# YushenLi807/WWW24-RAT

Measured on AMD Instinct MI355X. Metric: training samples/sec at B=4096, K=10 retrieved, d=64; 1/2/4/8 MI355X, higher is better.
Workload: dtype f32; 1 GPU; synthetic_F20_V1M_K10_d64_B4096; fields=20, vocab_rows=1000000, retrieved=10, embedding_dim=64, batch_per_gpu=4096, global_batch=4096, heads=8, dim_head=10, depth=4, scale_dim=2, step=fwd+bwd+clip+adam, embedding_grad=atomic, sync_batch_norm=False, parallelism=dp1

## Files before the change

www24-rat_amd/csrc/attn.hip:

```cpp
#include "rat_device.h"
#include "../../include/rat_hip.h"

#include <cstdlib>
#include <initializer_list>

namespace {

constexpr int ATT_THREADS = 512;
constexpr int ATT_WAVES = ATT_THREADS / 64;
constexpr int ATT_ROWS = 64;
constexpr int ATT_MT = ATT_ROWS / 16;
constexpr int DH_MAX = 16;
constexpr int QSLOTS = 8;
constexpr int OSLOTS = 4;
constexpr int FAST_INNER = 80;
constexpr int fast_heads(int tdh) { return tdh > 0 ? FAST_INNER / tdh : 0; }
constexpr int CORE_UNROLL = 3;

struct AttnArgs {
    const float* x;
    const float* dy;
    float* y;
    const float* res;
    const float* add;
    int add_lds;
    float out_scale;
    float* o_save;
    float* lse_save;
    const float* ln_g;
    const float* ln_b;
    const float* w_qkv;
    const float* w_out;
    const float* b_out;
    float* slabs;
    int64_t slab_stride;
    int64_t nseq, q_div, hi_stride, lo_stride, pos_stride;
    int64_t nchunks;
    int L, nsq_chunk;
    int nq;
    int d, heads, dh;
    float eps, scale;
    int vec_x, vec_wqkv, vec_wout;
    RatDrop drop;
    int groups;
    int64_t group_tok;
    unsigned long long* prof;
};

struct AttnGeom {
    int D, I, Q3, D16, I16, Q16, ldx, ldq, ldt;
    __host__ __device__ AttnGeom(int d, int heads, int dh) {
        D = d;
        I = heads * dh;
        Q3 = 3 * I;
        D16 = (D + 15) / 16 * 16;
        I16 = (I + 15) / 16 * 16;
        Q16 = (Q3 + 15) / 16 * 16;
        ldx = D16 + 4;
        ldq = Q16 + 4;
        ldt = (D16 > I16 ? D16 : I16) + 4;
    }
    size_t fwd_smem() const { return (size_t)ATT_ROWS * (ldx + ldq) * 4 + 2 * ATT_ROWS * 8; }
    size_t bwd_smem(int heads) const {
        return (size_t)ATT_ROWS * (2 * ldx + ldq + 2 * ldt) * 4 + (size_t)ATT_ROWS * (2 + 2 * heads) * 4 + 2 * ATT_ROWS * 8;
    }
    int64_t slab_floats() const { return (int64_t)Q3 * D + (int64_t)D * I + 3 * (int64_t)D; }
};

__device__ __forceinline__ int64_t seq_token(const AttnArgs& a, int64_t q, int p) {
    if (a.nseq <= 0x7fffffffLL && a.q_div <= 0x7fffffffLL) {
        const unsigned qq = (unsigned)q, dv = (unsigned)a.q_div, hi = qq / dv;
        return (int64_t)hi * a.hi_stride + (int64_t)(qq - hi * dv) * a.lo_stride + (int64_t)p * a.pos_stride;
    }
    return (q / a.q_div) * a.hi_stride + (q % a.q_div) * a.lo_stride + (int64_t)p * a.pos_stride;
}

__device__ __forceinline__ void map_rows(const AttnArgs& a, int64_t chunk, int64_t* rowtok, int& nsq, int& rows) {
    const int64_t q0 = chunk * a.nsq_chunk;
    const int64_t left = a.nseq - q0;
    nsq = left < a.nsq_chunk ? (int)left : a.nsq_chunk;
    rows = nsq * a.L;
    if (threadIdx.x < ATT_ROWS) {
        const int r = threadIdx.x;
        rowtok[r] = r < rows ? seq_token(a, q0 + r / a.L, r % a.L) : (int64_t)-1;
    }
// ... 935 lines not shown
    RAT_REQUIRE(d <= 128, "embedding_dim > 128 is not supported by this kernel");
    RAT_REQUIRE(map->L >= 1 && map->L <= ATT_ROWS, "sequence length (K+1 or F+1) must be in [1, 64]");
    RAT_REQUIRE(map->nseq >= 1 && map->q_div >= 1, "bad seq map");
    const AttnGeom g(d, heads, dim_head);
    RAT_REQUIRE(g.fwd_smem() <= 160 * 1024, "heads*dim_head too large for the LDS tile (forward)");
    if (backward) {
        RAT_REQUIRE(g.bwd_smem(heads) <= 160 * 1024, "heads*dim_head too large for the LDS tile (backward)");
        RAT_REQUIRE((g.Q16 / 16) * (g.D16 / 16) <= QSLOTS * ATT_WAVES,
                    "3*heads*dim_head x embedding_dim exceeds the in-register dW_qkv accumulator budget");
        RAT_REQUIRE((g.D16 / 16) * (g.I16 / 16) <= OSLOTS * ATT_WAVES,
                    "embedding_dim x heads*dim_head exceeds the in-register dW_out accumulator budget");
    }
    return 0;
}

bool aligned16(const void* p) { return (reinterpret_cast<uintptr_t>(p) & 15) == 0; }

void fill_common(AttnArgs& a, const RatAttnParams* w, const RatSeqMap* map, int d, int heads, int dim_head,
                 float ln_eps) {
    a.ln_g = w->ln_g;
    a.ln_b = w->ln_b;
    a.w_qkv = w->w_qkv;
    a.w_out = w->w_out;
    a.b_out = w->b_out;
    a.nseq = map->nseq;
    a.q_div = map->q_div;
    a.hi_stride = map->hi_stride;
    a.lo_stride = map->lo_stride;
    a.pos_stride = map->pos_stride;
    a.L = map->L;
    a.nq = (map->queries > 0 && map->queries < map->L) ? map->queries : map->L;
    a.nsq_chunk = ATT_ROWS / map->L;
    a.nchunks = (map->nseq + a.nsq_chunk - 1) / a.nsq_chunk;
    a.d = d;
    a.heads = heads;
    a.dh = dim_head;
    a.eps = ln_eps;
    a.scale = 1.0f / sqrtf((float)dim_head);
    a.out_scale = 1.0f;
    const int I = heads * dim_head;
    a.vec_wqkv = (d % 4 == 0) && aligned16(w->w_qkv);
    a.vec_wout = (I % 4 == 0) && aligned16(w->w_out);
    a.prof = rat_prof_buffer();
}

bool aligned8(const void* p) { return (reinterpret_cast<uintptr_t>(p) & 7) == 0; }

int fast_dim(const AttnArgs& a, std::initializer_list<const void*> ptrs) {
    if (!((a.dh == 10 || a.dh == 20) && a.heads == fast_heads(a.dh)) || a.w_out == nullptr) return 0;
    for (const void* p : ptrs)
        if (p != nullptr && !aligned16(p)) return 0;
    if (!aligned16(a.w_qkv) || !aligned16(a.w_out)) return 0;
    return (a.d == 64 || a.d == 16) ? a.d : 0;
}

}

extern "C" int rat_attn_fwd(const float* x, float* y, float* o_save, float* lse_save, const RatAttnParams* w_host,
                            const RatSeqMap* map_host, int d, int heads, int dim_head, float ln_eps, void* stream) {
    return rat_attn_fwd_ex(x, x, y, o_save, lse_save, w_host, map_host, d, heads, dim_head, 0.f, 1.f, ln_eps, 0.f, 0, RAT_ARITH_F32,
                           nullptr, 0, stream);
}

static bool b3_dim(int d) { return d == B3_D || d == 40 || d == 48 || d == 56; }
static bool b3_geom(int d, int heads, int dim_head) {
    return (b3_dim(d) && heads == B3_H && dim_head == B3_DH) || (d == B3_D && heads == 4 && dim_head == 2 * B3_DH);
}
static bool b3_shape(int d, int heads, int dim_head, const RatAttnParams* w) {
    return b3_geom(d, heads, dim_head) && w->w_out != nullptr;
}
static bool b3_ph_fits(int L, int nsq_chunk, int heads = B3_H) { return (size_t)nsq_chunk * heads * L * L * 4 <= (size_t)3 * B3_XP; }
static int b3_matrix_core(int L) {
    const int k = rat_knob(RAT_KNOB_ATTN_BWD_CORE_MFMA);
    if (L > 48 || k == 0) return 0;
    if (L > 32) return (k == 1 || L >= 40) ? 13 : 0;
    return (k == 1 || L >= 28) ? (L > 16 ? 2 : 1) : 0;
}
static int b3_fwd_matrix_core(int L, int nq) {
    const int k = rat_knob(RAT_KNOB_ATTN_FWD_CORE_MFMA);
    if (L > 48 || nq < L || k == 3) return 0;
    if (k != 2 && !((L >= 28 && L <= 32) || L >= 40)) return 0;
    return L > 32 ? 3 : (L > 16 ? 2 : 1);
}
static bool b3_ph_enabled() {
    return rat_knob(RAT_KNOB_ATTN_BWD_PH) != 0;
}
static int b3_nvalid(int d) { return d == B3_D ? 0 : d; }
static bool b3_off32_ok(const RatSeqMap* m) {
    if (m->hi_stride < 0 || m->lo_stride < 0 || m->pos_stride < 0) return false;
    const int64_t qd = m->q_div, hi = (m->nseq - 1) / qd, lo = m->nseq - 1 < qd - 1 ? m->nseq - 1 : qd - 1;
    const double max_tok = (double)hi * (double)m->hi_stride + (double)lo * (double)m->lo_stride + (double)(m->L - 1) * (double)m->pos_stride;
    return (max_tok + 1.0) * (double)(B3_I * 4) < 4294967296.0;
}

extern "C" size_t rat_attn_fwd_workspace(int d, int heads, int dim_head) {
    return b3_geom(d, heads, dim_head) ? B3_W_QKV + B3_W_OUT : 0;
}

extern "C" size_t rat_attn_planes_bytes(int d, int heads, int dim_head) {
    return b3_geom(d, heads, dim_head) ? B3_W_BYTES : 0;
}
extern "C" int rat_attn_split_jobs(const RatAttnParams* w_host, int d, int heads, int dim_head, void* planes, RatSplitJob* jobs_out) {
    RAT_REQUIRE(w_host && jobs_out, "null pointer");
    if (!b3_shape(d, heads, dim_head, w_host) || planes == nullptr) return 0;
    RAT_REQUIRE(aligned16(planes) && w_host->w_qkv, "planes must be 16-byte aligned");
    char* ws = static_cast<char*>(planes);
    jobs_out[0] = RatSplitJob{w_host->w_qkv, ws, B3_Q3, d, d, 0, 0, 0};
    jobs_out[1] = RatSplitJob{w_host->w_out, ws + B3_W_QKV, B3_I, d, B3_I, 1, 0, 0};
    jobs_out[2] = RatSplitJob{w_host->w_qkv, ws + B3_W_QKV + B3_W_OUTT, B3_D, B3_Q3, d, 1, 0, b3_nvalid(d)};
    jobs_out[3] = RatSplitJob{w_host->w_out, ws + B3_W_QKV + B3_W_OUTT + B3_W_QKVT, B3_D, B3_I, B3_I, 0, 0, b3_nvalid(d)};
    return 4;
}

extern "C" int rat_attn_fwd_ex(const float* x, const float* res, float* y, float* o_save, float* lse_save,
                               const RatAttnParams* w_host, const RatSeqMap* map_host, int d, int heads, int dim_head,
                               float softmax_scale, float out_scale, float ln_eps, float dropout_p, uint64_t dropout_seed,
                               int arith, float* workspace, size_t workspace_bytes, void* stream) {
    if (check_dims(map_host, d, heads, dim_head, false)) return -1;
    RAT_REQUIRE(x && y && w_host && w_host->ln_g && w_host->ln_b && w_host->w_qkv, "null pointer");
    RAT_REQUIRE(w_host->w_out != nullptr || heads * dim_head == d, "missing w_out");
    AttnArgs a{};
    fill_common(a, w_host, map_host, d, heads, dim_head, ln_eps);
    if (softmax_scale > 0.f) a.scale = softmax_scale;
    a.out_scale = out_scale;
    a.res = res;
    a.x = x;
    a.y = y;
    a.o_save = o_save;
    a.lse_save = lse_save;
    a.vec_x = (d % 4 == 0) && aligned16(x) && aligned16(y) && aligned16(res);
    const AttnGeom g(d, heads, dim_head);
    const bool ct_shape = dim_head == 10 && ((d == 10 && (heads == 8 || heads == 2)) || (d == 16 && heads == 2));
    const size_t smem = g.fwd_smem() + (ct_shape ? ct_weight_floats(g) * sizeof(float) : 0);
    const int per_cu = (int)((160 * 1024) / smem) >= 2 ? 2 : 1;
    const unsigned blocks = (unsigned)(a.nchunks < rat_max_blocks() * per_cu ? a.nchunks : rat_max_blocks() * per_cu);
    RAT_REQUIRE(dropout_p >= 0.f && dropout_p < 1.f, "dropout_p must be in [0, 1)");
    if (dropout_p > 0.f && w_host->w_out != nullptr)
        a.drop = RatDrop{dropout_seed, (uint32_t)((double)dropout_p * 4294967296.0), 1.0f / (1.0f - dropout_p), w_host->drop_seed_dev};
    const int fast = fast_dim(a, {x, y, res, o_save, lse_save});
    const bool plain = res == x && out_scale == 1.0f && a.drop.threshold == 0;
    const bool have_planes = w_host->planes != nullptr && aligned16(w_host->planes);
    const bool dpad = d != B3_D && b3_dim(d) && heads == fast_heads(dim_head) && aligned16(x) && aligned16(y) && aligned16(res) &&
                      aligned16(o_save) && aligned16(lse_save) && aligned16(w_host->w_qkv) && aligned16(w_host->w_out);
    if (arith == RAT_ARITH_BF16X3 && (fast == 64 || dpad) && b3_shape(d, heads, dim_head, w_host) && b3_off32_ok(map_host) &&
        (have_planes || (workspace != nullptr && workspace_bytes >= B3_W_QKV + B3_W_OUT && aligned16(workspace)))) {
        const char* p_qkv;
        const char* p_out;
        if (have_planes) {
            p_qkv = static_cast<const char*>(w_host->planes);
            p_out = p_qkv + B3_W_QKV + B3_W_OUTT + B3_W_QKVT;
        } else {
            char* ws = reinterpret_cast<char*>(workspace);
            if (rat_launch_split_weights(w_host->w_qkv, B3_Q3, d, d, 0, ws, stream) ||
                rat_launch_split_weights(w_host->w_out, B3_D, B3_I, B3_I, 0, ws + B3_W_QKV, stream, 0, b3_nvalid(d))) return -1;
            p_qkv = ws;
            p_out = ws + B3_W_QKV;
        }
        Attn3W W{};
        W.qkv = RatWPlanes{reinterpret_cast<const rat_u4*>(p_qkv), 2};
        W.out = RatWPlanes{reinterpret_cast<const rat_u4*>(p_out), 3};
        const unsigned b3_blocks = (unsigned)(a.nchunks < rat_max_blocks() ? a.nchunks : rat_max_blocks());
        if (heads == 4) {
            RAT_LAUNCH((attn_fwd3_kernel<true, false, false, false, 0, 4>), b3_blocks, ATT_THREADS, b3_fwd_smem(), stream, a, W);
            return rat_check_launch("rat_attn_fwd (bf16x3, 4 heads)");
        }
        if (dpad) {
            if (plain && a.nq < a.L) RAT_LAUNCH((attn_fwd3_kernel<false, true, true>), b3_blocks, ATT_THREADS, b3_fwd_smem(), stream, a, W);
            else if (plain) RAT_LAUNCH((attn_fwd3_kernel<false, false, true>), b3_blocks, ATT_THREADS, b3_fwd_smem(), stream, a, W);
            else RAT_LAUNCH((attn_fwd3_kernel<true, false, true>), b3_blocks, ATT_THREADS, b3_fwd_smem(), stream, a, W);
        } else if (plain && a.nq < a.L) RAT_LAUNCH((attn_fwd3_kernel<false, true>), b3_blocks, ATT_THREADS, b3_fwd_smem(), stream, a, W);
        else if (plain && b3_fwd_matrix_core(a.L, a.nq) == 3)
            RAT_LAUNCH((attn_fwd3_kernel<false, false, false, false, 3>), b3_blocks, ATT_THREADS, b3_fwd_smem(), stream, a, W);
        else if (plain && b3_fwd_matrix_core(a.L, a.nq) == 2)
            RAT_LAUNCH((attn_fwd3_kernel<false, false, false, false, 2>), b3_blocks, ATT_THREADS, b3_fwd_smem(), stream, a, W);
        else if (plain && b3_fwd_matrix_core(a.L, a.nq) == 1)
            RAT_LAUNCH((attn_fwd3_kernel<false, false, false, false, 1>), b3_blocks, ATT_THREADS, b3_fwd_smem(), stream, a, W);
        else if (plain) RAT_LAUNCH((attn_fwd3_kernel<false>), b3_blocks, ATT_THREADS, b3_fwd_smem(), stream, a, W);
        else if (b3_fwd_matrix_core(a.L, a.L) == 3)
            RAT_LAUNCH((attn_fwd3_kernel<true, false, false, false, 3>), b3_blocks, ATT_THREADS, b3_fwd_smem(), stream, a, W);
        else if (b3_fwd_matrix_core(a.L, a.L) == 2)
            RAT_LAUNCH((attn_fwd3_kernel<true, false, false, false, 2>), b3_blocks, ATT_THREADS, b3_fwd_smem(), stream, a, W);
        else RAT_LAUNCH((attn_fwd3_kernel<true>), b3_blocks, ATT_THREADS, b3_fwd_smem(), stream, a, W);
        return rat_check_launch("rat_attn_fwd (bf16x3)");
    }
    const bool head_vec = aligned8(o_save);
    RAT_REQUIRE(head_vec || dim_head <= DH_MAX, "o_save must be 8-byte aligned for dim_head 20");
    if (!head_vec) RAT_LAUNCH((attn_fwd_kernel<0, 0>), blocks, ATT_THREADS, smem, stream, a);
    else if (fast == 64 && dim_head == 10 && plain) RAT_LAUNCH((attn_fwd_kernel<64, 10, false>), blocks, ATT_THREADS, smem, stream, a);
    else if (fast == 64 && dim_head == 10) RAT_LAUNCH((attn_fwd_kernel<64, 10>), blocks, ATT_THREADS, smem, stream, a);
    else if (fast == 16 && dim_head == 10) RAT_LAUNCH((attn_fwd_kernel<16, 10>), blocks, ATT_THREADS, smem, stream, a);
    else if (fast == 64 && dim_head == 20) RAT_LAUNCH((attn_fwd_kernel<64, 20>), blocks, ATT_THREADS, smem, stream, a);
    else if (dim_head == 20) RAT_LAUNCH((attn_fwd_kernel<0, 20>), blocks, ATT_THREADS, smem, stream, a);
    else if (dim_head == 10 && d == 10 && heads == 8) RAT_LAUNCH((attn_fwd_kernel<0, 10, true, 2, 8, 10>), blocks, ATT_THREADS, smem, stream, a);
    else if (dim_head == 10 && d == 10 && heads == 2) RAT_LAUNCH((attn_fwd_kernel<0, 10, true, 2, 2, 10>), blocks, ATT_THREADS, smem, stream, a);
    else if (dim_head == 10 && d == 16 && heads == 2) RAT_LAUNCH((attn_fwd_kernel<0, 10, true, 2, 2, 16>), blocks, ATT_THREADS, smem, stream, a);
    else if (dim_head == 10 && d <= 16) RAT_LAUNCH((attn_fwd_kernel<0, 10, true, 2>), blocks, ATT_THREADS, smem, stream, a);
    else if (dim_head == 10) RAT_LAUNCH((attn_fwd_kernel<0, 10>), blocks, ATT_THREADS, smem, stream, a);
    else RAT_LAUNCH((attn_fwd_kernel<0, 0>), blocks, ATT_THREADS, smem, stream, a);
    return rat_check_launch("rat_attn_fwd");
}

static int b3_groups(int d, int heads, int dim_head) {
    return (d == B3_D && dim_head == B3_DH && heads > B3_H && heads % B3_H == 0 && heads / B3_H <= 8) ? heads / B3_H : 0;
}
static int wide_heads(int dim_head) { return dim_head == WG_DH ? WG_H : (dim_head == 2 * WG_DH ? WG_H / 2 : 0); }
static int wide_groups(int d, int heads, int dim_head) {
    const int wh = wide_heads(dim_head);
    return (d >= 1 && d <= 16 && wh > 0 && heads > wh && heads % wh == 0 && heads / wh <= 8) ? heads / wh : 0;
}
extern "C" int rat_attn_groups_supported(int d, int heads, int dim_head) {
    if (b3_groups(d, heads, dim_head)) return 1;
    const int G = wide_groups(d, heads, dim_head);
    return G == 0 ? 0 : (G <= WG_MAXG ? 3 : 1);
}
extern "C" size_t rat_attn_groups_planes_bytes(int d, int heads, int dim_head) {
    return (size_t)b3_groups(d, heads, dim_head) * B3_GRP_PLANES;
}
extern "C" int rat_attn_groups_split_jobs(const RatAttnParams* w_host, int d, int heads, int dim_head, void* planes, RatSplitJob* jobs_out) {
    RAT_REQUIRE(w_host && jobs_out, "null pointer");
    const int G = b3_groups(d, heads, dim_head);
    if (G == 0 || planes == nullptr || w_host->w_out == nullptr) return 0;
    RAT_REQUIRE(aligned16(planes) && w_host->w_qkv, "planes must be 16-byte aligned");
    const int I = heads * dim_head;
    int n = 0;
    const int rows = (B3_I << 8) | (I << 20);
    for (int g = 0; g < G; ++g) {
        char* ws = static_cast<char*>(planes) + (size_t)g * B3_GRP_PLANES;
        const float* wq = w_host->w_qkv + (size_t)g * B3_I * d;
        const float* wo = w_host->w_out + (size_t)g * B3_I;
        jobs_out[n++] = RatSplitJob{wq, ws, B3_Q3, d, d, 0, rows, 0};
        jobs_out[n++] = RatSplitJob{wo, ws + B3_W_QKV, B3_I, d, I, 1, 0, 0};
        jobs_out[n++] = RatSplitJob{wq, ws + B3_W_QKV + B3_W_OUTT, B3_D, B3_Q3, d, 1, rows, 0};
        jobs_out[n++] = RatSplitJob{wo, ws + B3_W_QKV + B3_W_OUTT + B3_W_QKVT, B3_D, B3_I, I, 0, 0, 0};
    }
    return n;
}
extern "C" int rat_attn_fwd_groups(const float* x, const float* res, float* y, float* o_save, float* lse_save, int64_t ntok,
                                   const RatAttnParams* w_host, const void* planes, const RatSeqMap* map_host, int d, int heads,
                                   int dim_head, float softmax_scale, float out_scale, float ln_eps, float dropout_p,
                                   uint64_t dropout_seed, void* stream) {
    const int Gw = wide_groups(d, heads, dim_head);
    if (Gw > 0) {
        const int wh = wide_heads(dim_head);
        if (check_dims(map_host, d, wh, dim_head, false)) return -1;
        RAT_REQUIRE(x && y && w_host && w_host->ln_g && w_host->ln_b && w_host->w_qkv && w_host->w_out && w_host->b_out, "null pointer");
        RAT_REQUIRE((o_save == nullptr) == (lse_save == nullptr) && ntok > 0, "o_save and lse_save come together, [G][ntok][.]");
        AttnArgs a{};
        fill_common(a, w_host, map_host, d, wh, dim_head, ln_eps);
        a.vec_wout = ((heads * dim_head) % 4 == 0) && aligned16(w_host->w_out);
        a.vec_wqkv = (aligned8(x) && aligned16(w_host->w_out)) ? 1 : 0;
        if (softmax_scale > 0.f) a.scale = softmax_scale;
        a.out_scale = out_scale;
        a.res = res;
        a.x = x;
        a.y = y;
        a.o_save = o_save;
        a.lse_save = lse_save;
        a.groups = Gw;
        a.group_tok = ntok;
        a.vec_x = (d % 4 == 0) && aligned16(x) && aligned16(y) && aligned16(res);
        RAT_REQUIRE(dropout_p >= 0.f && dropout_p < 1.f, "dropout_p must be in [0, 1)");
        if (dropout_p > 0.f)
            a.drop = RatDrop{dropout_seed, (uint32_t)((double)dropout_p * 4294967296.0), 1.0f / (1.0f - dropout_p), w_host->drop_seed_dev};
        const size_t smem = AttnGeom(d, wh, dim_head).fwd_smem() + (size_t)WG_WO_FLOATS * 4;
// ... 214 lines not shown
```

www24-rat_amd/csrc/attn_b3.h:

```cpp
constexpr int B3_D = 64, B3_I = 80, B3_Q3 = 240, B3_H = 8, B3_DH = 10;
constexpr int B3_LDQ = B3_Q3 + 4;
constexpr int B3_XP = 64 * 128;
constexpr int B3_OP = 64 * 160 + 64;
constexpr int B3_QP = 64 * 480;
typedef RatPlanes<128, 7, B3_XP> PlanesX;
typedef RatPlanes<160, 0, B3_OP> PlanesO;
typedef RatPlanes<480, 0, B3_QP> PlanesQ;

struct Attn3W {
    RatWPlanes qkv;
    RatWPlanes out;
    RatWPlanes outT;
    RatWPlanes qkvT;
};
constexpr size_t B3_W_QKV = (size_t)15 * 2 * 3 * 1024, B3_W_OUT = (size_t)4 * 3 * 3 * 1024, B3_W_OUTT = (size_t)5 * 2 * 3 * 1024,
                 B3_W_QKVT = (size_t)4 * 8 * 3 * 1024;
constexpr size_t B3_W_BYTES = B3_W_QKV + B3_W_OUT + B3_W_OUTT + B3_W_QKVT;

constexpr size_t B3_FWD_LSE = (size_t)3 * B3_XP + (size_t)64 * B3_LDQ * 4 + (size_t)3 * B3_OP + 2 * 64 * 8;
constexpr size_t B3_FWD_WOUT = B3_FWD_LSE + (size_t)64 * B3_H * 4;
constexpr size_t b3_fwd_smem() { return B3_FWD_WOUT + B3_W_OUT; }
constexpr size_t B3_GRP_PLANES = B3_W_BYTES;
static_assert(b3_fwd_smem() <= 160 * 1024, "LDS budget (forward)");
struct RatWPlanesLds {
// ... 325 lines not shown
            }
            for (; j < L; ++j) {
                const float* kp = kbase + (size_t)j * B3_LDQ;
                kv.load(kp, NDH);
                const float sv = q.dot(kv) * sl2;
                const float mn = fmaxf(m, sv);
                const float corr = rat_exp2(m - mn);
                const float p = rat_exp2(sv - mn);
                l = l * corr + p;
                kv.load(kp + B3_I, NDH);
                o.scale_axpy(corr, p, kv);
                m = mn;
            }
            const float inv = 1.0f / l;
            o.store(qp, NDH, inv);
            lse_s[row_i * NH + h] = m + rat_log2(l);
        }
        if (QSUB && nq < L) {
            for (int e = threadIdx.x; e < rows * NH; e += ATT_THREADS) {
                const int r = e / NH, h = e - r * NH;
                if (r % L < nq) continue;
                HV z;
                z.zero();
                z.store(qkv + (size_t)r * B3_LDQ + h * NDH, NDH, 1.0f);
                lse_s[e] = 0.f;
            }
        }
        __syncthreads();
        RAT_PROF_MARK(2);
        for (int e = threadIdx.x; e < ATT_ROWS * (B3_I / 8); e += ATT_THREADS) {
            const int r = e / (B3_I / 8), o8 = e - r * (B3_I / 8);
            const float* src = qkv + (size_t)r * B3_LDQ + 8 * o8;
            const float4 v0 = *reinterpret_cast<const float4*>(src), v1 = *reinterpret_cast<const float4*>(src + 4);
            rat_u4 h, m, l;
            rat_split8(v0, v1, h, m, l);
            op.store(r, o8, h, m, l);
            const int64_t tok = rowtok[r];
            if (o_save != nullptr && tok >= 0) {
                rat_st4_stream(o_save + tok * B3_I + 8 * o8, v0);
                rat_st4_stream(o_save + tok * B3_I + 8 * o8 + 4, v1);
            }
        }
        if (lse_save != nullptr && (int)threadIdx.x < (NH / 4) * ATT_ROWS) {
            const int r = threadIdx.x / (NH / 4), part = threadIdx.x % (NH / 4);
            const int64_t tok = rowtok[r];
            if (tok >= 0) rat_st4_stream(lse_save + tok * NH + 4 * part, *reinterpret_cast<const float4*>(lse_s + r * NH + 4 * part));
        }
        __syncthreads();
        RAT_PROF_MARK(3);
        if (GRP) {
            b3_gemm_rows<3>(op, wo, B3_D / 16, [&](int mt, int nt, const f32x4& acc) {
#pragma unroll
                for (int r = 0; r < 4; ++r) yacc[mt & 1][r] += acc[r];
            });
            continue;
        }
        b3_gemm_rows<3>(op, wout_lds, B3_D / 16, [&](int mt, int nt, const f32x4& acc) {
            const int col = rat_acc_col(nt);
            const float bias = (!DPAD || col < dreal) ? a.b_out[col] : 0.f;
#pragma unroll
            for (int r = 0; r < 4; ++r) ys[(size_t)rat_acc_row(mt, r) * LDY + col] = acc[r] + bias;
        });
        }
        if (GRP) {
            const int w = rat_wave(), col = rat_acc_col(w & 3);
            const float bias = a.b_out[col];
#pragma unroll
            for (int i = 0; i < 2; ++i)
#pragma unroll
                for (int r = 0; r < 4; ++r) ys[(size_t)rat_acc_row(2 * (w >> 2) + i, r) * LDY + col] = yacc[i][r] + bias;
        }
        __syncthreads();
        RAT_PROF_MARK(4);
        if (EX) {
            store_rows_residual(a.y, ys, LDY, a.res, rowtok, rows, dreal, true, a.out_scale, &a.drop);
        } else {
            const int r = threadIdx.x >> 3, sb = threadIdx.x & 7;
            const int64_t tok = rowtok[r];
            if (tok >= 0 && colok) {
                const float4 t0 = *reinterpret_cast<const float4*>(ys + (size_t)r * LDY + 8 * sb);
                const float4 t1 = *reinterpret_cast<const float4*>(ys + (size_t)r * LDY + 8 * sb + 4);
                *reinterpret_cast<float4*>(a.y + tok * dreal + 8 * sb) = make_float4(t0.x + x0.x, t0.y + x0.y, t0.z + x0.z, t0.w + x0.w);
                *reinterpret_cast<float4*>(a.y + tok * dreal + 8 * sb + 4) = make_float4(t1.x + x1.x, t1.y + x1.y, t1.z + x1.z, t1.w + x1.w);
            }
        }
        __syncthreads();
#ifndef RAT_EMU
        asm volatile("" ::"v"(pf));
#endif
        RAT_PROF_MARK(5);
    }
    RAT_PROF_FLUSH(a.prof, 48);
}

constexpr int B3_LDT = B3_I + 4;
constexpr int B3_LDN = B3_D + 4;
constexpr size_t B3_OFF_DYP = (size_t)3 * B3_XP, B3_OFF_QKV = 2 * B3_OFF_DYP, B3_OFF_OB = B3_OFF_QKV + (size_t)64 * B3_LDQ * 4,
                 B3_OFF_DOB = B3_OFF_OB + (size_t)64 * B3_LDT * 4, B3_OFF_MISC = B3_OFF_DOB + (size_t)64 * B3_LDT * 4;
constexpr size_t b3_bwd_smem() { return B3_OFF_MISC + (size_t)64 * (2 + 2 * B3_H) * 4 + 2 * 64 * 8 + 2 * B3_D * 4; }
static_assert(B3_OFF_MISC - B3_OFF_QKV >= (size_t)3 * B3_QP + 64, "d(Q|K|V) planes overlay the three fp32 tiles");
static_assert((size_t)64 * B3_LDN * 4 <= (size_t)3 * B3_XP, "d(LN out) overlays the dy planes");

template <int KS, class PA, class Epi>
__device__ __forceinline__ void b3_gemm_rows_longk(const PA& A, const RatWPlanes& Bw, const Epi& epi) {
    const int w = rat_wave(), mt0 = 2 * (w >> 2), nt = w & 3;
    f32x4 acc[2] = {rat_zero4(), rat_zero4()};
    RatB3 b = Bw(nt, 0);
    RatB3 a[2] = {A.row_frag(mt0, 0), A.row_frag(mt0 + 1, 0)};
#pragma unroll
    for (int s = 0; s < KS; ++s) {
        const int sn = s + 1 < KS ? s + 1 : s;
        const RatB3 bn = Bw(nt, sn);
        const RatB3 an[2] = {A.row_frag(mt0, sn), A.row_frag(mt0 + 1, sn)};
        rat_mfma3_block<2>(acc, a, b);
        a[0] = an[0];
        a[1] = an[1];
        b = bn;
    }
    epi(mt0, nt, acc[0]);
    epi(mt0 + 1, nt, acc[1]);
}

template <int NIT>
__device__ __forceinline__ void b3_bwd_core_mfma(float* qkv, float* ob, const float* dob, const float* lses, float* scratch, int L, int nsq,
                                                 float scale) {
    constexpr int SLD = 16 * NIT + 1, SCR = 16 * SLD + 16;
    const int w = rat_wave(), l = rat_lane(), g = l >> 4, m = l & 15;
    float* scr = scratch + w * SCR;
    float* dl = scr + 16 * SLD;
    const float sl2 = scale * RAT_LOG2E;
    const int npairs = nsq * B3_H;
    const bool cm = m < B3_DH;
    const int mc = m;
    for (int pair = w; pair < npairs; pair += ATT_WAVES) {
        const int h = pair % B3_H, sq = pair / B3_H;
        const int r0 = sq * L, cq = h * B3_DH, ck = B3_I + h * B3_DH, cv = 2 * B3_I + h * B3_DH;
        f32x4 adK[NIT], adV[NIT];
#pragma unroll
        for (int jt = 0; jt < NIT; ++jt) adK[jt] = adV[jt] = rat_zero4();
#pragma unroll
        for (int it = 0; it < NIT; ++it) {
            const int i0 = 16 * it;
            const int irows = L - i0 < 16 ? L - i0 : 16;
            {
                const int rr = r0 + i0 + m;
                const float* a_ = dob + (size_t)rr * B3_LDT + cq;
                const float* b_ = ob + (size_t)rr * B3_LDT + cq;
                float d = 0.f;
#pragma unroll
                for (int c = 0; c < B3_DH; c += 2) {
                    const float2 x = *reinterpret_cast<const float2*>(a_ + c), y = *reinterpret_cast<const float2*>(b_ + c);
                    d = fmaf(x.x, y.x, d);
                    d = fmaf(x.y, y.y, d);
                }
                if (l < 16) dl[l] = m < irows ? d : 0.f;
            }
            float aq[3], ao[3], bk[3][NIT], bv[3][NIT];
            const int ri = r0 + i0 + m;
#pragma unroll
            for (int ks = 0; ks < 3; ++ks) {
                const int cc = 4 * ks + g;
                aq[ks] = qkv[(size_t)ri * B3_LDQ + cq + cc];
                ao[ks] = dob[(size_t)ri * B3_LDT + cq + cc];
#pragma unroll
                for (int jt = 0; jt < NIT; ++jt) {
                    const int rj = r0 + 16 * jt + m;
// ... 613 lines not shown
```

www24-rat_amd/csrc/rat_common.hip:

```cpp
#include "rat_device.h"
#include <stdlib.h>
#include <vector>
#include "../../include/rat_hip.h"

static thread_local std::string g_last_error;

const char* rat_set_error(const std::string& msg) {
    g_last_error = msg;
    return g_last_error.c_str();
}
int rat_fail(const std::string& msg) {
    rat_set_error(msg);
    return -1;
}
int rat_check_launch(const char* what) {
    hipError_t e = hipGetLastError();
    if (e != hipSuccess) return rat_fail(std::string(what) + ": " + hipGetErrorString(e));
    return 0;
}

static int g_knobs[RAT_KNOB_COUNT];
static const char* const g_knob_names[RAT_KNOB_COUNT] = {"max_blocks", "attn_bwd_ph", "attn_fwd_core_mfma", "attn_bwd_core_mfma", "ffn_bwd_t3",
                                                         "sgemm_split_target"};
static const bool g_knobs_loaded = [] {
    auto env = [](const char* n) { const char* e = getenv(n); return e ? std::string(e) : std::string(); };
    const std::string mb = env("RAT_MAX_BLOCKS"), ph = env("RAT_ATTN_BWD_PH"), fc = env("RAT_ATTN_FWD_CORE"), bc = env("RAT_ATTN_BWD_CORE"),
                      ff = env("RAT_FFN_BWD"), st = env("RAT_SGEMM_SPLIT_TARGET");
    g_knobs[RAT_KNOB_MAX_BLOCKS] = mb.empty() ? 0 : atoi(mb.c_str());
    g_knobs[RAT_KNOB_ATTN_BWD_PH] = (ph.empty() || ph[0] != '0') ? 1 : 0;
    g_knobs[RAT_KNOB_ATTN_FWD_CORE_MFMA] = fc == "mfma" ? 1 : (fc == "mfma32" ? 2 : (fc == "valu" ? 3 : 0));
    g_knobs[RAT_KNOB_ATTN_BWD_CORE_MFMA] = bc == "mfma" ? 1 : (bc == "valu" ? 0 : -1);
    g_knobs[RAT_KNOB_FFN_BWD_T3] = ff.rfind("t3", 0) == 0 ? 1 : 0;
    g_knobs[RAT_KNOB_SGEMM_SPLIT_TARGET] = st.empty() ? 0 : (atoi(st.c_str()) > 0 ? atoi(st.c_str()) : 0);
    return true;
}();
int rat_knob(int which) { return g_knobs[which]; }
extern "C" int rat_debug_set_knob(const char* name, int value) {
    for (int i = 0; i < RAT_KNOB_COUNT; ++i)
        if (name != nullptr && std::string(name) == g_knob_names[i]) {
            const int old = g_knobs[i];
            g_knobs[i] = value;
            return old;
        }
    return -2147483647 - 1;
}
int rat_max_blocks() {
    const int n = g_knobs[RAT_KNOB_MAX_BLOCKS];
    return n > 0 && n < 256 ? n : 256;
}

static unsigned long long* g_prof = nullptr;
unsigned long long* rat_prof_buffer() { return g_prof; }
extern "C" void rat_debug_set_prof(void* device_u64x64) { g_prof = static_cast<unsigned long long*>(device_u64x64); }

extern "C" int rat_version(void) { return RAT_ABI_VERSION; }
extern "C" const char* rat_last_error(void) { return g_last_error.c_str(); }

struct RatReduceArgs {
    const float* slabs;
    int nslabs;
    int64_t stride;
    int nouts;
    float* out[8];
    int64_t off[8];
    int64_t size[8];
    int64_t first_block[9];
};

__global__ void __launch_bounds__(256) rat_reduce_slabs_kernel(RatReduceArgs r) {
    __shared__ float part[256];
    int o = 0;
    while (o + 1 < r.nouts && (int64_t)blockIdx.x >= r.first_block[o + 1]) ++o;
    const int lane_p = threadIdx.x & 63, quarter = threadIdx.x >> 6;
    const int64_t p = ((int64_t)blockIdx.x - r.first_block[o]) * 64 + lane_p;
    float s = 0.f;
    if (p < r.size[o]) {
        const int per = (r.nslabs + 3) / 4;
        const int w0 = quarter * per, w1 = (w0 + per < r.nslabs) ? w0 + per : r.nslabs;
        const float* src = r.slabs + r.off[o] + p;
        int w = w0;
        for (; w + 8 <= w1; w += 8) {
            float v[8];
#pragma unroll
            for (int k = 0; k < 8; ++k) v[k] = src[(int64_t)(w + k) * r.stride];
#pragma unroll
            for (int k = 0; k < 8; ++k) s += v[k];
        }
        for (; w < w1; ++w) s += src[(int64_t)w * r.stride];
    }
    part[threadIdx.x] = s;
    __syncthreads();
    if (quarter == 0 && p < r.size[o]) r.out[o][p] = ((part[lane_p] + part[64 + lane_p]) + part[128 + lane_p]) + part[192 + lane_p];
}

struct RatReduceEntry {
    const float* src;
    float* out;
    int64_t size, stride;
    int nslabs, first_block;
};
constexpr int RAT_REDUCE_BATCH = 80;
struct RatReduceTable {
    RatReduceEntry e[RAT_REDUCE_BATCH];
    int n, blocks;
};
static thread_local bool g_defer = false;
static thread_local std::vector<RatReduceEntry> g_deferred;

__global__ void __launch_bounds__(256) rat_reduce_slabs_batch_kernel(RatReduceTable t) {
    __shared__ float4 part4[256];
    float* part = reinterpret_cast<float*>(part4);
    int o = 0;
    auto first = [&](int i) { const int f = t.e[i].first_block; return f < 0 ? -f - 1 : f; };
    while (o + 1 < t.n && (int)blockIdx.x >= first(o + 1)) ++o;
    const RatReduceEntry& r = t.e[o];
    const bool vec = r.first_block < 0;
// ... 219 lines not shown
```

www24-rat_amd/csrc/rat_device.h:

```cpp
#pragma once

#include <stdint.h>
#include <stddef.h>

#ifdef RAT_EMU
#include "hip_emu.h"
#define RAT_MFMA16(a, b, c) emu_mfma_f32_16x16x4f32((a), (b), (c))
#define RAT_MFMA4(a, b, c) emu_mfma_f32_4x4x1f32((a), (b), (c))
#else
#include <hip/hip_runtime.h>
typedef float f32x4 __attribute__((vector_size(16)));
#define RAT_MFMA16(a, b, c) __builtin_amdgcn_mfma_f32_16x16x4f32((a), (b), (c), 0, 0, 0)
#define RAT_MFMA4(a, b, c) __builtin_amdgcn_mfma_f32_4x4x1f32((a), (b), (c), 0, 0, 0)
#define RAT_LAUNCH(kernel, grid, block, smem, stream, ...) \
    hipLaunchKernelGGL(kernel, dim3(grid), dim3(block), (smem), (hipStream_t)(stream), __VA_ARGS__)
#define RAT_DYN_SMEM(name) extern __shared__ __attribute__((aligned(16))) char name[]
#endif

#include <string>

#if defined(RAT_PROF) && !defined(RAT_EMU)
#define RAT_PROF_DECL unsigned long long prof_t0 = clock64(); unsigned long long prof_acc[12] = {0, 0, 0, 0, 0, 0, 0, 0, 0, 0, 0, 0};
#define RAT_PROF_MARK(i) do { const unsigned long long prof_t = clock64(); prof_acc[i] += prof_t - prof_t0; prof_t0 = prof_t; } while (0)
#define RAT_PROF_FLUSH(ptr, base) do { if (threadIdx.x == 0 && (ptr) != nullptr) for (int pi = 0; pi < 12; ++pi) atomicAdd((ptr) + (base) + pi, prof_acc[pi]); } while (0)
#define RAT_TRACE(ptr, on, slot) do { if ((ptr) != nullptr && (on) && blockIdx.x == 0 && (threadIdx.x & 63) == 0) (ptr)[256 + (threadIdx.x >> 6) * 32 + (slot)] = clock64(); } while (0)
#else
#define RAT_PROF_DECL
#define RAT_PROF_MARK(i) do { } while (0)
#define RAT_PROF_FLUSH(ptr, base) do { } while (0)
#define RAT_TRACE(ptr, on, slot) do { } while (0)
#endif
#ifdef RAT_EMU
#define RAT_WAVE_FENCE() emu::wave_sync()
#else
#define RAT_WAVE_FENCE() do { __builtin_amdgcn_fence(__ATOMIC_ACQ_REL, "wavefront"); __builtin_amdgcn_wave_barrier(); } while (0)
#endif
unsigned long long* rat_prof_buffer();

const char* rat_set_error(const std::string& msg);
int rat_fail(const std::string& msg);
int rat_check_launch(const char* what);
enum { RAT_KNOB_MAX_BLOCKS, RAT_KNOB_ATTN_BWD_PH, RAT_KNOB_ATTN_FWD_CORE_MFMA, RAT_KNOB_ATTN_BWD_CORE_MFMA, RAT_KNOB_FFN_BWD_T3,
       RAT_KNOB_SGEMM_SPLIT_TARGET, RAT_KNOB_COUNT };
int rat_knob(int which);
int rat_max_blocks();

#define RAT_REQUIRE(cond, msg)                  \
    do {                                        \
        if (!(cond)) return rat_fail(std::string(__func__) + ": " + (msg)); \
    } while (0)

static inline int rat_round_up(int v, int m) { return (v + m - 1) / m * m; }

#define RAT_WAVE 64
#ifdef RAT_EMU
#define RAT_SCHED_FENCE() do { } while (0)
#define RAT_SCHED_MFMA_VALU(n, v) do { } while (0)
#else
#define RAT_SCHED_FENCE() __builtin_amdgcn_sched_barrier(0)
#define RAT_SCHED_MFMA_VALU(n, v)                                   \
    do {                                                            \
        _Pragma("unroll") for (int sgb_i = 0; sgb_i < (n); ++sgb_i) { \
            __builtin_amdgcn_sched_group_barrier(0x008, 1, 0);      \
            __builtin_amdgcn_sched_group_barrier(0x002, (v), 0);    \
        }                                                           \
    } while (0)
#endif

__device__ __forceinline__ int rat_lane() { return threadIdx.x & 63; }
#ifdef RAT_EMU
__device__ __forceinline__ int rat_wave() { return threadIdx.x >> 6; }
#else
__device__ __forceinline__ int rat_wave() { return __builtin_amdgcn_readfirstlane((int)(threadIdx.x >> 6)); }
#endif

__device__ __forceinline__ float4 rat_consume4(const float4& src) {
#ifdef RAT_EMU
    return src;
#else
    float4 d;
    asm volatile("v_mov_b32 %0, %4\n\tv_mov_b32 %1, %5\n\tv_mov_b32 %2, %6\n\tv_mov_b32 %3, %7"
                 : "=&v"(d.x), "=&v"(d.y), "=&v"(d.z), "=&v"(d.w)
                 : "v"(src.x), "v"(src.y), "v"(src.z), "v"(src.w));
    return d;
#endif
}

__device__ __forceinline__ uint32_t rat_hash32(uint64_t seed, uint64_t i) {
    uint64_t z = seed + 0x9E3779B97F4A7C15ull * (i + 1);
    z = (z ^ (z >> 30)) * 0xBF58476D1CE4E5B9ull;
    z = (z ^ (z >> 27)) * 0x94D049BB133111EBull;
    z = z ^ (z >> 31);
    return (uint32_t)(z >> 32);
}
struct RatDrop {
    uint64_t seed;
    uint32_t threshold;
    float scale;
    const uint64_t* seed_dev;
    __device__ __forceinline__ uint64_t the_seed() const { return seed_dev != nullptr ? *seed_dev : seed; }
    __device__ __forceinline__ float apply(float v, int64_t idx) const {
        return threshold == 0 ? v : (rat_hash32(the_seed(), (uint64_t)idx) >= threshold ? v * scale : 0.f);
    }
};

__device__ __forceinline__ void rat_st4_stream(float* p, const float4& v) {
#ifdef RAT_EMU
    *reinterpret_cast<float4*>(p) = v;
#else
    const f32x4 t = {v.x, v.y, v.z, v.w};
    __builtin_nontemporal_store(t, reinterpret_cast<f32x4*>(p));
#endif
}
__device__ __forceinline__ float4 rat_ld4_stream(const float* p) {
#ifdef RAT_EMU
    return *reinterpret_cast<const float4*>(p);
#else
    const f32x4 t = __builtin_nontemporal_load(reinterpret_cast<const f32x4*>(p));
    return make_float4(t[0], t[1], t[2], t[3]);
#endif
}

__device__ __forceinline__ f32x4 rat_zero4() {
    f32x4 z = {0.f, 0.f, 0.f, 0.f};
    return z;
}
// ... 509 lines not shown
```

Baseline: 225,100 samples/s.

## Add two-workgroup-per-CU attention forward kernel with reduced LDS footprint

Adds a variant of the bf16x3 attention forward kernel that packs the Q, K|V, O and staging buffers into overlapping LDS regions under an 80 KB budget. It sets launch bounds so two 512-thread work-groups can be resident per CU, and launches up to twice as many blocks. The QKV GEMM keeps its A fragments in registers and releases the LDS before the epilogue, so the outputs can overwrite the x planes. The goal is better latency hiding through higher occupancy, at the cost of register pressure and extra overlay hazards. A knob enables it by default, and a launch counter is added for debugging.

```diff
diff --git a/www24-rat_amd/csrc/attn.hip b/www24-rat_amd/csrc/attn.hip
--- a/www24-rat_amd/csrc/attn.hip
+++ b/www24-rat_amd/csrc/attn.hip
@@ -1,6 +1,7 @@
 #include "rat_device.h"
 #include "../../include/rat_hip.h"
 
+#include <atomic>
 #include <cstdlib>
 #include <initializer_list>
 
@@ -1102,6 +1103,9 @@
     if (k != 2 && !((L >= 28 && L <= 32) || L >= 40)) return 0;
     return L > 32 ? 3 : (L > 16 ? 2 : 1);
 }
+static bool b3_fwd_two_groups() { return rat_knob(RAT_KNOB_ATTN_FWD_2WG) != 0; }
+static std::atomic<long long> g_fwd3_2wg_launches{0};
+extern "C" long long rat_debug_attn_fwd_2wg_launches(void) { return g_fwd3_2wg_launches.load(std::memory_order_relaxed); }
 static bool b3_ph_enabled() {
     return rat_knob(RAT_KNOB_ATTN_BWD_PH) != 0;
 }
@@ -1180,6 +1184,7 @@
         W.qkv = RatWPlanes{reinterpret_cast<const rat_u4*>(p_qkv), 2};
         W.out = RatWPlanes{reinterpret_cast<const rat_u4*>(p_out), 3};
         const unsigned b3_blocks = (unsigned)(a.nchunks < rat_max_blocks() ? a.nchunks : rat_max_blocks());
+        const unsigned b3_blocks2 = (unsigned)(a.nchunks < 2 * rat_max_blocks() ? a.nchunks : 2 * rat_max_blocks());
         if (heads == 4) {
             RAT_LAUNCH((attn_fwd3_kernel<true, false, false, false, 0, 4>), b3_blocks, ATT_THREADS, b3_fwd_smem(), stream, a, W);
             return rat_check_launch("rat_attn_fwd (bf16x3, 4 heads)");
@@ -1195,11 +1200,19 @@
             RAT_LAUNCH((attn_fwd3_kernel<false, false, false, false, 2>), b3_blocks, ATT_THREADS, b3_fwd_smem(), stream, a, W);
         else if (plain && b3_fwd_matrix_core(a.L, a.nq) == 1)
             RAT_LAUNCH((attn_fwd3_kernel<false, false, false, false, 1>), b3_blocks, ATT_THREADS, b3_fwd_smem(), stream, a, W);
+        else if (plain && b3_fwd_two_groups()) {
+            RAT_LAUNCH((attn_fwd3_2wg_kernel<false>), b3_blocks2, ATT_THREADS, b3_fwd2_smem(), stream, a, W);
+            g_fwd3_2wg_launches.fetch_add(1, std::memory_order_relaxed);
+        }
         else if (plain) RAT_LAUNCH((attn_fwd3_kernel<false>), b3_blocks, ATT_THREADS, b3_fwd_smem(), stream, a, W);
         else if (b3_fwd_matrix_core(a.L, a.L) == 3)
             RAT_LAUNCH((attn_fwd3_kernel<true, false, false, false, 3>), b3_blocks, ATT_THREADS, b3_fwd_smem(), stream, a, W);
         else if (b3_fwd_matrix_core(a.L, a.L) == 2)
             RAT_LAUNCH((attn_fwd3_kernel<true, false, false, false, 2>), b3_blocks, ATT_THREADS, b3_fwd_smem(), stream, a, W);
+        else if (b3_fwd_two_groups()) {
+            RAT_LAUNCH((attn_fwd3_2wg_kernel<true>), b3_blocks2, ATT_THREADS, b3_fwd2_smem(), stream, a, W);
+            g_fwd3_2wg_launches.fetch_add(1, std::memory_order_relaxed);
+        }
         else RAT_LAUNCH((attn_fwd3_kernel<true>), b3_blocks, ATT_THREADS, b3_fwd_smem(), stream, a, W);
         return rat_check_launch("rat_attn_fwd (bf16x3)");
     }
diff --git a/www24-rat_amd/csrc/attn_b3.h b/www24-rat_amd/csrc/attn_b3.h
--- a/www24-rat_amd/csrc/attn_b3.h
+++ b/www24-rat_amd/csrc/attn_b3.h
@@ -431,6 +431,236 @@
                 const float4 t1 = *reinterpret_cast<const float4*>(ys + (size_t)r * LDY + 8 * sb + 4);
                 *reinterpret_cast<float4*>(a.y + tok * dreal + 8 * sb) = make_float4(t0.x + x0.x, t0.y + x0.y, t0.z + x0.z, t0.w + x0.w);
                 *reinterpret_cast<float4*>(a.y + tok * dreal + 8 * sb + 4) = make_float4(t1.x + x1.x, t1.y + x1.y, t1.z + x1.z, t1.w + x1.w);
+            }
+        }
+        __syncthreads();
+#ifndef RAT_EMU
+        asm volatile("" ::"v"(pf));
+#endif
+        RAT_PROF_MARK(5);
+    }
+    RAT_PROF_FLUSH(a.prof, 48);
+}
+
+constexpr int B3_LDQ2 = B3_I + 4;
+constexpr int B3_LDK2 = 2 * B3_I + 4;
+constexpr size_t B3_F2_KV = (size_t)3 * B3_XP, B3_F2_MAP = B3_F2_KV + (size_t)64 * B3_LDK2 * 4, B3_F2_LSE = B3_F2_MAP + 2 * 64 * 8,
+                 B3_F2_LN = B3_F2_LSE + (size_t)64 * B3_H * 4;
+constexpr size_t b3_fwd2_smem() { return B3_F2_LN + 2 * B3_D * 4; }
+static_assert(b3_fwd2_smem() <= 80 * 1024, "LDS budget (forward, two work-groups per CU)");
+static_assert((size_t)64 * B3_LDQ2 * 4 <= B3_F2_KV && (size_t)64 * (B3_D + 4) * 4 <= B3_F2_KV, "fp32 Q / the staging tile overlay the x planes");
+static_assert((size_t)3 * B3_OP <= (size_t)64 * B3_LDK2 * 4, "the O planes overlay the K|V tile");
+
+template <int KS, class PA, class BW, class Epi>
+__device__ __forceinline__ void b3_gemm_rows_release(const PA& A, const BW& Bw, int n_tiles, const Epi& epi) {
+    const int w = rat_wave(), mt0 = 2 * (w >> 2);
+    int nt = w & 3;
+    RatB3 b = Bw(nt, 0);
+    RatB3 a[2][KS];
+#pragma unroll
+    for (int i = 0; i < 2; ++i)
+#pragma unroll
+        for (int s = 0; s < KS; ++s) a[i][s] = A.row_frag(mt0 + i, s);
+    __syncthreads();
+    for (; nt < n_tiles; nt += 4) {
+        f32x4 acc[2] = {rat_zero4(), rat_zero4()};
+#pragma unroll
+        for (int s = 0; s < KS; ++s) {
+            const bool last = s == KS - 1;
+            const RatB3 bn = Bw(last ? (nt + 4 < n_tiles ? nt + 4 : nt) : nt, last ? 0 : s + 1);
+            const RatB3 as[2] = {a[0][s], a[1][s]};
+            rat_mfma3_block<2>(acc, as, b);
+            b = bn;
+        }
+        epi(mt0, nt, acc[0]);
+        epi(mt0 + 1, nt, acc[1]);
+    }
+}
+
+template <int KS, class PA, class BW, class Epi>
+__device__ __forceinline__ void b3_gemm_rows_stream(const PA& A, const BW& Bw, int n_tiles, const Epi& epi) {
+    const int w = rat_wave(), mt0 = 2 * (w >> 2);
+    int nt = w & 3;
+    if (nt >= n_tiles) return;
+    RatB3 b = Bw(nt, 0);
+    for (; nt < n_tiles; nt += 4) {
+        f32x4 acc[2] = {rat_zero4(), rat_zero4()};
+#pragma unroll
+        for (int s = 0; s < KS; ++s) {
+            const bool last = s == KS - 1;
+            const RatB3 bn = Bw(last ? (nt + 4 < n_tiles ? nt + 4 : nt) : nt, last ? 0 : s + 1);
+            const RatB3 as[2] = {A.row_frag(mt0, s), A.row_frag(mt0 + 1, s)};
+            rat_mfma3_block<2>(acc, as, b);
+            b = bn;
+        }
+        epi(mt0, nt, acc[0]);
+        epi(mt0 + 1, nt, acc[1]);
+    }
+}
+
+__device__ __forceinline__ int b3_tid_here() {
+    int t = threadIdx.x;
+#ifndef RAT_EMU
+    asm volatile("" : "+v"(t));
+#endif
+    return t;
+}
+
+template <bool EX>
+__global__ void __launch_bounds__(ATT_THREADS, 4) attn_fwd3_2wg_kernel(AttnArgs a, Attn3W W) {
+    RAT_DYN_SMEM(smem);
+    const PlanesX xp{smem};
+    float* const qs = reinterpret_cast<float*>(smem);
+    float* const ys = reinterpret_cast<float*>(smem);
+    float* const kv = reinterpret_cast<float*>(smem + B3_F2_KV);
+    const PlanesO op{smem + B3_F2_KV};
+    int64_t* const rowtok0 = reinterpret_cast<int64_t*>(smem + B3_F2_MAP);
+    float* const lse_s = reinterpret_cast<float*>(smem + B3_F2_LSE);
+    float* const ln_s = reinterpret_cast<float*>(smem + B3_F2_LN);
+    constexpr int LDY = B3_D + 4;
+    const int L = a.L;
+    if ((int)threadIdx.x < 2 * B3_D) ln_s[threadIdx.x] = (int)threadIdx.x < B3_D ? a.ln_g[threadIdx.x] : a.ln_b[threadIdx.x - B3_D];
+    {
+        int nsq0, rows0;
+        map_rows(a, blockIdx.x, rowtok0, nsq0, rows0);
+    }
+    __syncthreads();
+    RAT_PROF_DECL
+    int parity = 0;
+    for (int64_t chunk = blockIdx.x; chunk < a.nchunks; chunk += gridDim.x, parity ^= 1) {
+        const int64_t* rowtok = rowtok0 + parity * ATT_ROWS;
+        int nsq, rows;
+        {
+            const int64_t q0 = chunk * a.nsq_chunk;
+            const int64_t left = a.nseq - q0;
+            nsq = left < a.nsq_chunk ? (int)left : a.nsq_chunk;
+            rows = nsq * a.L;
+        }
+        float4 x0, x1;
+        b3_load_piece(a.x, rowtok, x0, x1);
+        {
+            float gam[8], bet[8];
+            const float4 g0 = *reinterpret_cast<const float4*>(ln_s + 8 * (threadIdx.x & 7)), g1 = *reinterpret_cast<const float4*>(ln_s + 8 * (threadIdx.x & 7) + 4);
+            const float4 b0 = *reinterpret_cast<const float4*>(ln_s + B3_D + 8 * (threadIdx.x & 7)), b1 = *reinterpret_cast<const float4*>(ln_s + B3_D + 8 * (threadIdx.x & 7) + 4);
+            gam[0] = g0.x; gam[1] = g0.y; gam[2] = g0.z; gam[3] = g0.w; gam[4] = g1.x; gam[5] = g1.y; gam[6] = g1.z; gam[7] = g1.w;
+            bet[0] = b0.x; bet[1] = b0.y; bet[2] = b0.z; bet[3] = b0.w; bet[4] = b1.x; bet[5] = b1.y; bet[6] = b1.z; bet[7] = b1.w;
+            b3_layer_norm_to_planes<false>(rowtok[threadIdx.x >> 3] >= 0, x0, x1, a.eps, xp, gam, bet, nullptr, nullptr);
+        }
+        if (chunk + gridDim.x < a.nchunks) {
+            int nsq1, rows1;
+            map_rows(a, chunk + gridDim.x, (rowtok0 + (parity ^ 1) * ATT_ROWS), nsq1, rows1);
+        }
+        __syncthreads();
+        RAT_PROF_MARK(0);
+        b3_gemm_rows_release<2>(xp, W.qkv, B3_Q3 / 16, [&](int mt, int nt, const f32x4& acc) {
+            const int col = rat_acc_col(nt);
+            float* const dst = nt < B3_I / 16 ? qs + col : kv + (col - B3_I);
+            const int ld = nt < B3_I / 16 ? B3_LDQ2 : B3_LDK2;
+#pragma unroll
+            for (int r = 0; r < 4; ++r) dst[(size_t)rat_acc_row(mt, r) * ld] = acc[r];
+        });
+        __syncthreads();
+        RAT_PROF_MARK(1);
+        float pf = 0.f;
+        int tid = b3_tid_here();
+        if (tid < ATT_ROWS * 2 && chunk + gridDim.x < a.nchunks)
+            pf = prefetch_lines_map((rowtok0 + (parity ^ 1) * ATT_ROWS), tid, 2, a.x, B3_D);
+        typedef HeadVec<B3_DH> HV;
+        const int ntasks = nsq * B3_H * L;
+        const float sl2 = a.scale * RAT_LOG2E;
+        for (int task = tid; task < ntasks; task += ATT_THREADS) {
+            const int i = task % L;
+            const int h = (task / L) % B3_H;
+            const int sq = task / (L * B3_H);
+            const int row_i = sq * L + i;
+            float* qp = qs + (size_t)row_i * B3_LDQ2 + h * B3_DH;
+            HV q, o, kk1;
+            q.load(qp, B3_DH);
+            o.zero();
+            float m = -INFINITY, l = 0.f;
+            const float* kbase = kv + (size_t)(sq * L) * B3_LDK2 + h * B3_DH;
+            int j = 0;
+            for (; j + CORE_UNROLL <= L; j += CORE_UNROLL) {
+                HV kk[CORE_UNROLL], vv[CORE_UNROLL];
+#pragma unroll
+                for (int u = 0; u < CORE_UNROLL; ++u) {
+                    const float* kp = kbase + (size_t)(j + u) * B3_LDK2;
+                    kk[u].load(kp, B3_DH);
+                    vv[u].load(kp + B3_I, B3_DH);
+                }
+                float sc[CORE_UNROLL];
+#pragma unroll
+                for (int u = 0; u < CORE_UNROLL; ++u) sc[u] = q.dot(kk[u]) * sl2;
+#pragma unroll
+                for (int u = 0; u < CORE_UNROLL; ++u) {
+                    const float mn = fmaxf(m, sc[u]);
+                    const float corr = rat_exp2(m - mn);
+                    const float p = rat_exp2(sc[u] - mn);
+                    l = l * corr + p;
+                    o.scale_axpy(corr, p, vv[u]);
+                    m = mn;
+                }
+            }
+            for (; j < L; ++j) {
+                const float* kp = kbase + (size_t)j * B3_LDK2;
+                kk1.load(kp, B3_DH);
+                const float sv = q.dot(kk1) * sl2;
+                const float mn = fmaxf(m, sv);
+                const float corr = rat_exp2(m - mn);
+                const float p = rat_exp2(sv - mn);
+                l = l * corr + p;
+                kk1.load(kp + B3_I, B3_DH);
+                o.scale_axpy(corr, p, kk1);
+                m = mn;
+            }
+            const float inv = 1.0f / l;
+            o.store(qp, B3_DH, inv);
+            lse_s[row_i * B3_H + h] = m + rat_log2(l);
+        }
+        __syncthreads();
+        RAT_PROF_MARK(2);
+        tid = b3_tid_here();
+        if (tid < 3 * 16)
+            *reinterpret_cast<float*>(op.base + (size_t)(tid >> 4) * B3_OP + 64 * 160 + 4 * (tid & 15)) = 0.f;
+        for (int e = tid; e < ATT_ROWS * (B3_I / 8); e += ATT_THREADS) {
+            const int r = e / (B3_I / 8), o8 = e - r * (B3_I / 8);
+            const float* src = qs + (size_t)r * B3_LDQ2 + 8 * o8;
+            const float4 v0 = *reinterpret_cast<const float4*>(src), v1 = *reinterpret_cast<const float4*>(src + 4);
+            rat_u4 h, m, l;
+            rat_split8(v0, v1, h, m, l);
+            op.store(r, o8, h, m, l);
+            const int64_t tok = rowtok[r];
+            if (a.o_save != nullptr && tok >= 0) {
+                rat_st4_stream(a.o_save + tok * B3_I + 8 * o8, v0);
+                rat_st4_stream(a.o_save + tok * B3_I + 8 * o8 + 4, v1);
+            }
+        }
+        if (a.lse_save != nullptr && tid < (B3_H / 4) * ATT_ROWS) {
+            const int r = tid / (B3_H / 4), part = tid % (B3_H / 4);
+            const int64_t tok = rowtok[r];
+            if (tok >= 0) rat_st4_stream(a.lse_save + tok * B3_H + 4 * part, *reinterpret_cast<const float4*>(lse_s + r * B3_H + 4 * part));
+        }
+        __syncthreads();
+        RAT_PROF_MARK(3);
+        b3_gemm_rows_stream<3>(op, W.out, B3_D / 16, [&](int mt, int nt, const f32x4& acc) {
+            const int col = rat_acc_col(nt);
+            const float bias = a.b_out[col];
+#pragma unroll
+            for (int r = 0; r < 4; ++r) ys[(size_t)rat_acc_row(mt, r) * LDY + col] = acc[r] + bias;
+        });
+        __syncthreads();
+        RAT_PROF_MARK(4);
+        if (EX) {
+            store_rows_residual(a.y, ys, LDY, a.res, rowtok, rows, B3_D, true, a.out_scale, &a.drop);
+        } else {
+            tid = b3_tid_here();
+            const int r = tid >> 3, sb = tid & 7;
+            const int64_t tok = rowtok[r];
+            if (tok >= 0) {
+                const float4 t0 = *reinterpret_cast<const float4*>(ys + (size_t)r * LDY + 8 * sb);
+                const float4 t1 = *reinterpret_cast<const float4*>(ys + (size_t)r * LDY + 8 * sb + 4);
+                *reinterpret_cast<float4*>(a.y + tok * B3_D + 8 * sb) = make_float4(t0.x + x0.x, t0.y + x0.y, t0.z + x0.z, t0.w + x0.w);
+                *reinterpret_cast<float4*>(a.y + tok * B3_D + 8 * sb + 4) = make_float4(t1.x + x1.x, t1.y + x1.y, t1.z + x1.z, t1.w + x1.w);
             }
         }
         __syncthreads();
diff --git a/www24-rat_amd/csrc/rat_common.hip b/www24-rat_amd/csrc/rat_common.hip
--- a/www24-rat_amd/csrc/rat_common.hip
+++ b/www24-rat_amd/csrc/rat_common.hip
@@ -21,17 +21,18 @@
 
 static int g_knobs[RAT_KNOB_COUNT];
 static const char* const g_knob_names[RAT_KNOB_COUNT] = {"max_blocks", "attn_bwd_ph", "attn_fwd_core_mfma", "attn_bwd_core_mfma", "ffn_bwd_t3",
-                                                         "sgemm_split_target"};
+                                                         "sgemm_split_target", "attn_fwd_2wg"};
 static const bool g_knobs_loaded = [] {
     auto env = [](const char* n) { const char* e = getenv(n); return e ? std::string(e) : std::string(); };
     const std::string mb = env("RAT_MAX_BLOCKS"), ph = env("RAT_ATTN_BWD_PH"), fc = env("RAT_ATTN_FWD_CORE"), bc = env("RAT_ATTN_BWD_CORE"),
-                      ff = env("RAT_FFN_BWD"), st = env("RAT_SGEMM_SPLIT_TARGET");
+                      ff = env("RAT_FFN_BWD"), st = env("RAT_SGEMM_SPLIT_TARGET"), f2 = env("RAT_ATTN_FWD_2WG");
     g_knobs[RAT_KNOB_MAX_BLOCKS] = mb.empty() ? 0 : atoi(mb.c_str());
     g_knobs[RAT_KNOB_ATTN_BWD_PH] = (ph.empty() || ph[0] != '0') ? 1 : 0;
     g_knobs[RAT_KNOB_ATTN_FWD_CORE_MFMA] = fc == "mfma" ? 1 : (fc == "mfma32" ? 2 : (fc == "valu" ? 3 : 0));
     g_knobs[RAT_KNOB_ATTN_BWD_CORE_MFMA] = bc == "mfma" ? 1 : (bc == "valu" ? 0 : -1);
     g_knobs[RAT_KNOB_FFN_BWD_T3] = ff.rfind("t3", 0) == 0 ? 1 : 0;
     g_knobs[RAT_KNOB_SGEMM_SPLIT_TARGET] = st.empty() ? 0 : (atoi(st.c_str()) > 0 ? atoi(st.c_str()) : 0);
+    g_knobs[RAT_KNOB_ATTN_FWD_2WG] = f2.empty() ? -1 : (f2[0] == '0' ? 0 : 1);
     return true;
 }();
 int rat_knob(int which) { return g_knobs[which]; }
diff --git a/www24-rat_amd/csrc/rat_device.h b/www24-rat_amd/csrc/rat_device.h
--- a/www24-rat_amd/csrc/rat_device.h
+++ b/www24-rat_amd/csrc/rat_device.h
@@ -41,7 +41,7 @@
 int rat_fail(const std::string& msg);
 int rat_check_launch(const char* what);
 enum { RAT_KNOB_MAX_BLOCKS, RAT_KNOB_ATTN_BWD_PH, RAT_KNOB_ATTN_FWD_CORE_MFMA, RAT_KNOB_ATTN_BWD_CORE_MFMA, RAT_KNOB_FFN_BWD_T3,
-       RAT_KNOB_SGEMM_SPLIT_TARGET, RAT_KNOB_COUNT };
+       RAT_KNOB_SGEMM_SPLIT_TARGET, RAT_KNOB_ATTN_FWD_2WG, RAT_KNOB_COUNT };
 int rat_knob(int which);
 int rat_max_blocks();
 
```

New measurement: 229,200 samples/s (median of 6 runs). 1.8% higher.
